# arnaucube/go-snark-study

Hardware: AMD Instinct MI355X
Metric: Groth16 constraints/sec (prove) at 2^20 R1CS (higher is better)
Workload: dtype u32 (9x29-bit Montgomery limbs of the 254-bit BN128 fields)

## Files before the change

### __graft_entry__.py

```python
import os
import subprocess
import sys

ROOT = os.path.dirname(os.path.abspath(__file__))
if ROOT not in sys.path:
    sys.path.insert(0, ROOT)
TESTS = os.path.join(ROOT, "tests")


def build():
    jobs = str(min(8, os.cpu_count() or 1))
    subprocess.check_call(["make", "-s", "-j", jobs, "-C", os.path.join(ROOT, "go-snark-study_amd", "csrc")])
    subprocess.check_call(["make", "-s", "-C", os.path.join(ROOT, "oracle")])
    prim_src = os.path.join(ROOT, "tests", "device", "prim_test.hip")
    prim_lib = os.path.join(ROOT, "tests", "device", "libgs_prim_test.so")
    hdrs = [os.path.join(ROOT, "go-snark-study_amd", "csrc", h) for h in ("fp29.h", "fq2.h", "ec.h", "point_io.h")]
    hdrs.append(os.path.join(ROOT, "tests", "device", "limit_ops.h"))
    if not os.path.exists(prim_lib) or os.path.getmtime(prim_lib) < max(os.path.getmtime(f) for f in [prim_src] + hdrs):
        subprocess.check_call(["hipcc", "--offload-arch=gfx950", "-O3", "-std=c++17", "-fPIC", "-shared", "-Wno-unused-function", prim_src, "-o", prim_lib])
    if os.path.isdir("/root/reference"):
        subprocess.check_call(["make", "-s", "-C", os.path.join(ROOT, "oracle"), "ref"])
    import gosnark_amd
    from gosnark_amd import capi
    capi.load_library()
    _stamp_build()
    return None


def _stamp_build():
    import hashlib
    import json
    lib = os.path.join(ROOT, "go-snark-study_amd", "libgosnark_hip.so")
    info = {"lib_sha256": hashlib.sha256(open(lib, "rb").read()).hexdigest()}
    try:
        info["commit"] = subprocess.check_output(["git", "-C", ROOT, "rev-parse", "HEAD"], stderr=subprocess.DEVNULL).decode().strip()
        dirty = subprocess.check_output(["git", "-C", ROOT, "status", "--porcelain", "--", "go-snark-study_amd/csrc", "include"],
                                        stderr=subprocess.DEVNULL).decode()
        info["sources_modified_since_commit"] = sorted(line[3:] for line in dirty.splitlines() if len(line) > 3)
    except (OSError, subprocess.CalledProcessError):
        return
    with open(os.path.join(ROOT, "go-snark-study_amd", "BUILD_INFO.json"), "w") as f:
        json.dump(info, f, indent=1)


def smoke():
    import numpy as np
    import torch
    assert torch.cuda.is_available(), "smoke() needs a GPU"
    torch.cuda.set_device(0)
    if TESTS not in sys.path:
        sys.path.insert(0, TESTS)
    import gosnark_amd
    from gosnark_amd import capi, groth16
    capi.init(0)
    import golden_util as GU
    import gpu_util as U
    from oracle import c_oracle as C
    from oracle import ref_py as O
    rec = GU.load("groth_x3")
    opk = GU.groth_pk(rec["setup"])
    r, s = GU.rs_from_stream(rec["rand"])
    circ = groth16.Circuit(rec["circuit"]["NVars"], rec["circuit"]["NPublic"])
    pk = groth16.Pk(BACDelta=opk.BACDelta, Z=opk.Z, G1_Alpha=opk.G1_Alpha, G1_Beta=opk.G1_Beta, G1_Delta=opk.G1_Delta,
                    G1_At=opk.G1_At, G1_BACGamma=opk.G1_BACGamma, G2_Beta=opk.G2_Beta, G2_Delta=opk.G2_Delta,
                    G2_BACGamma=opk.G2_BACGamma, PowersTauDelta=opk.PowersTauDelta)
    proof = groth16.GenerateProofsWithRS(circ, pk, rec["w"], rec["px"], r, s)
    a = O.G1.Affine(GU.g1(rec["proof"]["PiA"]))
    b = O.G2.Affine(GU.g2(rec["proof"]["PiB"]))
    c = O.G1.Affine(GU.g1(rec["proof"]["PiC"]))
    assert proof.PiA == (a[0], a[1], 1), "PiA differs from the reference prover"
    assert proof.PiB == (b[0], b[1], (1, 0)), "PiB differs from the reference prover"
    assert proof.PiC == (c[0], c[1], 1), "PiC differs from the reference prover"
    n = 4096
    ks = U.rand_scalars_u64(n, 11)
    bases = capi.g1_fixed_base(ks)
    pts = capi.g1_download(bases)
    sc = U.rand_scalars_u64(n, 12)
    got = capi.msm(bases, sc)
    want = C.g1_affine(C.g1_msm_naive(pts, sc, threads=min(8, os.cpu_count() or 1)))
    assert got == want, "G1 MSM (table-free route) differs from the oracle's naive MulScalar/Add loop"
    capi.build_tables(bases)
    assert capi.handle_bytes(bases)[1] > 0 and capi.msm(bases, sc) == want, "G1 MSM (window-table route) differs from the oracle"
    proof2 = groth16.GenerateProofsWithRS(circ, pk, rec["w"], rec["px"], r, s)
    assert (proof2.PiA, proof2.PiB, proof2.PiC) == (proof.PiA, proof.PiB, proof.PiC)
    print("smoke ok: groth16 x^3+x+5 proof == reference wasm proof (affine); 4096-term G1 MSM == oracle on both summation routes;",
          capi.version())
    return None


if __name__ == "__main__":
    build()
    if len(sys.argv) > 1 and sys.argv[1] == "smoke":
        smoke()
```

### go-snark-study_amd/csrc/msm.hip

```cpp
#include "msm.h"
#include "hostcopy.h"

#include <algorithm>
#include <cmath>
#include <cstdlib>
#include <future>
#include <type_traits>

#include "msm_kernels.h"

namespace gs {

static_assert(sizeof(G1Xyzz) == PointIO<FqTag>::kXyzzWords * 4, "G1 XYZZ must be raw limbs");
static_assert(sizeof(G2Xyzz) == PointIO<Fq2Tag>::kXyzzWords * 4, "G2 XYZZ must be raw limbs");

static inline dim3 grid1(size_t n, int block = 256) { return dim3((unsigned)((n + block - 1) / block)); }

int choose_window_bits(uint32_t n, int forced) {
  if (forced >= 8 && forced <= kMaxWindowBits) return forced;
  static const double per_bucket = dev_knob_f("GS_WINDOW_COST_BUCKET", 6.0, 0.0, 64.0);
  static const int auto_max = (int)dev_knob("GS_AUTO_MAX_C", 17, 8, kMaxWindowBits);
  int best = 8;
  double best_cost = 1e300;
  for (int c = 8; c <= std::min(kMaxWindowBits, std::max(8, auto_max)); ++c) {
    const int W = 254 / c + 1;
    const double cost = (double)n * W + per_bucket * (double)(1u << (c - 1));
    if (cost < best_cost) { best_cost = cost; best = c; }
  }
  return best;
}

int choose_window_bits_free(uint32_t n, int forced) {
  if (forced) return std::min(kMaxFreeWindowBits, std::max(kMinFreeWindowBits, forced));
  static const double per_bucket = dev_knob_f("GS_WINDOW_COST_BUCKET_FREE", 3.0, 0.0, 64.0);
  int best = kMinFreeWindowBits;
  double best_cost = 1e300;
  for (int c = kMinFreeWindowBits; c <= kMaxFreeWindowBits; ++c) {
    const int W = 254 / c + 1;
    const double cost = (double)W * ((double)n + per_bucket * (double)(1u << (c - 1)));
    if (cost < best_cost) { best_cost = cost; best = c; }
  }
  return best;
}

static void exclusive_scan(Ctx& c, PlanBuffers& pb, const uint32_t* in, uint32_t* out, uint32_t n) {
  const uint32_t ntiles = (n + kScanTile - 1) / kScanTile;
  pb.tiles.ensure((size_t)ntiles * 4);
  pb.total.ensure(4);
  hipLaunchKernelGGL(k_scan_tiles, dim3(ntiles), dim3(kScanBlock), 0, c.stream, in, out, pb.tiles.as<uint32_t>(), n);
  hipLaunchKernelGGL(k_scan_tile_sums, dim3(1), dim3(1024), 0, c.stream, pb.tiles.as<uint32_t>(), ntiles, pb.total.as<uint32_t>());
  hipLaunchKernelGGL(k_scan_add, dim3(ntiles), dim3(kScanBlock), 0, c.stream, out, pb.tiles.as<uint32_t>(), n);
}

struct MsmState {
  PlanBuffers plan_slots[3 * Ctx::kSlots];
  DevBuf table_scratch;
  DevBuf table_scratch_bg;
  DevBuf upload_scratch;
  DevBuf upload_flag;
  bool lds_attr_set = false;
};
static MsmState& msm_state(Ctx& c) { return c.state<MsmState>(c.msm_state); }

static uint32_t choose_chunk(uint64_t entries, uint32_t nbuckets, const std::vector<LaunchShape>& users) {
  static const int forced = (int)dev_knob("GS_CHUNK", 0, 4, 1024, 4);
  if (forced >= 4 && forced % 4 == 0) return (uint32_t)forced;
  static const int forced_h = (int)dev_knob("GS_CHUNK_H", 0, 4, 1024, 4);
  if (forced_h && users.size() == 1 && users[0].njobs == 1 && !users[0].g2) return (uint32_t)forced_h;
  uint32_t chunk = entries >= (1ull << 27) ? 64u : entries >= (1ull << 23) ? 32u : 16u;
  while (chunk < 1024u && entries / std::max<uint32_t>(nbuckets, 1u) > 32ull * chunk) chunk *= 2;
  return chunk;
}

static uint32_t part_min_ranges() {
  static const uint32_t v = (uint32_t)dev_knob("GS_PART_MIN_R", 4, 2, 64);
  return v;
}
bool plan_partitions_first(int cbits) {
  if (cbits < 1) return false;
  return std::max<uint32_t>(1u, (1u << (cbits - 1)) >> kRangeLog) >= part_min_ranges();
}

uint32_t finite_mask_dev(Ctx& c, const uint32_t* g1_pts, const uint32_t* g2_pts, uint32_t n, uint32_t* mask_dev) {
  const size_t words = ((size_t)n + 31) / 32;
  GS_HIP(hipMemsetAsync(mask_dev, 0, std::max<size_t>(words, 1) * 4, c.stream));
  DevBuf cnt(4);
  GS_HIP(hipMemsetAsync(cnt.p, 0, 4, c.stream));
  if (n) hipLaunchKernelGGL(k_finite_mask, grid1(n), dim3(256), 0, c.stream, g1_pts, (uint32_t)PointIO<FqTag>::kAffineWords, g2_pts,
                            (uint32_t)PointIO<Fq2Tag>::kAffineWords, n, mask_dev, cnt.as<uint32_t>());
  GS_HIP(hipGetLastError());
  uint32_t host = 0;
  GS_HIP(hipMemcpyAsync(&host, cnt.p, 4, hipMemcpyDeviceToHost, c.stream));
  GS_HIP(hipStreamSynchronize(c.stream));
  return host;
}

void build_plan(Ctx& c, int slot, const uint32_t* scalars_dev, uint32_t n, MsmPlan& plan, const std::vector<LaunchShape>& users, int cbits,
                bool table_free, const uint32_t* term_index, uint32_t index_bias) {
  MsmState& ms = msm_state(c);
  PlanBuffers& pb = ms.plan_slots[slot % (3 * Ctx::kSlots)];
  plan.n = n;
  plan.table_free = table_free;
  plan.c = cbits ? cbits : (table_free ? choose_window_bits_free(n, c.window_bits) : choose_window_bits(n, c.window_bits));
  if (table_free && (plan.c < kMinFreeWindowBits || plan.c > kMaxFreeWindowBits))
    throw HipError{hipErrorInvalidValue, "table-free plan outside 9..16 window bits", __LINE__};
  plan.W = 254 / plan.c + 1;
  plan.B = 1u << (plan.c - 1);
  plan.nbuckets = table_free ? (uint32_t)plan.W * plan.B : plan.B;
  plan.chunk = choose_chunk((uint64_t)n * plan.W, plan.nbuckets, users);
  plan.maxchunks = (uint32_t)(((size_t)n * plan.W + plan.chunk - 1) / plan.chunk) + 1;
  const size_t ncount = (size_t)plan.nbuckets + 1;
  PlanParams pp{};
  pp.n = n; pp.c = plan.c; pp.W = plan.W; pp.B = plan.B;
  pp.R = std::max<uint32_t>(1u, plan.B >> kRangeLog);
  pp.tf = table_free ? 1u : 0u;
  {
    const uint32_t want = std::max<uint32_t>(1u, 256u / (plan.W * pp.R));
    const uint32_t by_size = std::max<uint32_t>(1u, (n + 16383u) / 16384u);
    const uint32_t by_mem = std::max<uint32_t>(1u, (uint32_t)((64ull << 20) / ((uint64_t)plan.B * plan.W * 4)));
    pp.S = std::max<uint32_t>(1u, std::min(std::min<uint32_t>(16u, std::max<uint32_t>(want, 1u)), std::min(by_size, by_mem)));
    if (pp.R == 1 && !table_free) pp.S = std::max<uint32_t>(1u, std::min<uint32_t>(16u, by_size));
  }
  pp.slice = (n + pp.S - 1) / pp.S;
  pp.stride = (n + 63u) & ~63u;
  const bool wide = plan_partitions_first(plan.c);
  if (wide && term_index) throw HipError{hipErrorInvalidValue, "plans over a term list cannot be sorted partition-first (plan_partitions_first)", __LINE__};
  const uint32_t nparts = (uint32_t)plan.W * pp.R;
  if (wide && nparts > kMaxParts) throw HipError{hipErrorInvalidValue, "too many (window, range) partitions", __LINE__};
  if (!wide) pb.digits.ensure((size_t)std::max<uint32_t>(pp.stride, 64u) * plan.W * sizeof(digit_t));
  else {
    pb.recs.ensure(std::max<size_t>((size_t)n * plan.W, 1) * 8);
    pb.parts.ensure((size_t)(3 * kMaxParts + 4) * 4);
  }
  pb.hist.ensure((size_t)plan.B * plan.W * pp.S * 4);
  pb.totals.ensure(ncount * 4);
  pb.offsets.ensure(ncount * 4);
  pb.entries.ensure(((size_t)plan.maxchunks + 1) * plan.chunk * 4);
  pb.chunk_bucket.ensure((size_t)plan.maxchunks * 4);
  pb.heavy_list.ensure((size_t)plan.nbuckets * 4);
  pb.counters.ensure(16);
  const size_t lds = (size_t)std::min<uint32_t>(plan.B, kRangeBuckets) * 4;
  static const int sort_block = (int)dev_knob("GS_SORT_BLOCK", kSortBlock, 64, kSortBlock, 64);
  if (!ms.lds_attr_set) {
    GS_HIP(hipFuncSetAttribute(reinterpret_cast<const void*>(k_hist), hipFuncAttributeMaxDynamicSharedMemorySize, 128 * 1024));
    GS_HIP(hipFuncSetAttribute(reinterpret_cast<const void*>(k_scatter), hipFuncAttributeMaxDynamicSharedMemorySize, 128 * 1024));
    GS_HIP(hipFuncSetAttribute(reinterpret_cast<const void*>(k_hist_part), hipFuncAttributeMaxDynamicSharedMemorySize, 128 * 1024));
    GS_HIP(hipFuncSetAttribute(reinterpret_cast<const void*>(k_scatter_part), hipFuncAttributeMaxDynamicSharedMemorySize, 128 * 1024));
    ms.lds_attr_set = true;
  }
  GS_HIP(hipMemsetAsync(pb.totals.as<uint32_t>() + plan.nbuckets, 0, 4, c.stream));
  GS_HIP(hipMemsetAsync(pb.counters.p, 0, 16, c.stream));
  uint32_t* part_count = pb.parts.as<uint32_t>();
  uint32_t* part_base = part_count ? part_count + kMaxParts : nullptr;
  uint32_t* part_cursor = part_count ? part_base + kMaxParts + 4 : nullptr;
  if (n > 0 && wide) {
    GS_HIP(hipMemsetAsync(part_count, 0, (size_t)nparts * 4, c.stream));
    hipLaunchKernelGGL(k_part_count, grid1(n, kPartBlock), dim3(kPartBlock), 0, c.stream, scalars_dev, pp, part_count);
    hipLaunchKernelGGL(k_part_scan, dim3(1), dim3(64), 0, c.stream, part_count, nparts, part_base, part_cursor);
    hipLaunchKernelGGL(k_part_scatter, grid1(n, kPartBlock * kPartPerThread), dim3(kPartBlock), 0, c.stream, scalars_dev, pp, part_base, part_cursor,
                       pb.recs.as<uint2>());
    hipLaunchKernelGGL(k_hist_part, dim3(8 * pp.S * ((nparts + 7) / 8)), dim3(sort_block), lds, c.stream, pb.recs.as<uint2>(), part_base, pp, pb.hist.as<uint32_t>());
    hipLaunchKernelGGL(k_colscan, grid1(plan.B), dim3(256), 0, c.stream, pb.hist.as<uint32_t>(), pp, pb.totals.as<uint32_t>());
  } else if (n > 0) {
    hipLaunchKernelGGL(k_digits, grid1(n), dim3(256), 0, c.stream, scalars_dev, pp, pb.digits.as<digit_t>(), term_index, index_bias);
    hipLaunchKernelGGL(k_hist, dim3(plan.W, pp.S, pp.R), dim3(sort_block), lds, c.stream, pb.digits.as<digit_t>(), pp, pb.hist.as<uint32_t>());
    if (table_free) hipLaunchKernelGGL(k_colscan_windows, grid1(plan.nbuckets), dim3(256), 0, c.stream, pb.hist.as<uint32_t>(), pp, pb.totals.as<uint32_t>());
    else hipLaunchKernelGGL(k_colscan, grid1(plan.B), dim3(256), 0, c.stream, pb.hist.as<uint32_t>(), pp, pb.totals.as<uint32_t>());
  } else {
    GS_HIP(hipMemsetAsync(pb.totals.p, 0, ncount * 4, c.stream));
  }
  exclusive_scan(c, pb, pb.totals.as<uint32_t>(), pb.offsets.as<uint32_t>(), (uint32_t)ncount);
  if (n > 0) {
    if (wide) hipLaunchKernelGGL(k_scatter_part, dim3(8 * pp.S * ((nparts + 7) / 8)), dim3(sort_block), lds, c.stream, pb.recs.as<uint2>(), part_base, pp,
                                 pb.hist.as<uint32_t>(), pb.offsets.as<uint32_t>(), pb.entries.as<uint32_t>());
    else hipLaunchKernelGGL(k_scatter, dim3(plan.W, pp.S, pp.R), dim3(sort_block), lds, c.stream, pb.digits.as<digit_t>(), pp, pb.hist.as<uint32_t>(),
                            pb.offsets.as<uint32_t>(), pb.entries.as<uint32_t>(), term_index, index_bias);
    hipLaunchKernelGGL(k_chunk_map, grid1(plan.nbuckets), dim3(256), 0, c.stream, pb.offsets.as<uint32_t>(), plan.nbuckets, plan.chunk,
                       pb.chunk_bucket.as<uint32_t>(), pb.heavy_list.as<uint32_t>(), pb.counters.as<uint32_t>());
  }
  GS_HIP(hipGetLastError());
  plan.offsets = pb.offsets.as<uint32_t>();
  plan.entries = pb.entries.as<uint32_t>();
  plan.chunk_bucket = pb.chunk_bucket.as<uint32_t>();
  plan.heavy_list = pb.heavy_list.as<uint32_t>();
  plan.heavy_count = pb.counters.as<uint32_t>();
}

template <class T>
static void enqueue_table_slabs(hipStream_t stream, DevBuf& scratch, const uint32_t* src, size_t n, int cbits, DevBuf& rows, size_t first, size_t last,
                                size_t slab) {
  const int W = 254 / cbits + 1;
  if (first >= last) return;
  static const bool per_row = dev_flag("GS_TABLE_PER_ROW");
  if (per_row || W <= 2) {
    if (first == 0) hipLaunchKernelGGL(k_build_table<T>, grid1(n), dim3(256), 0, stream, src, (uint32_t)n, cbits, W, rows.as<uint32_t>());
  } else {
    constexpr size_t sw = PointIO<T>::kXyzzWords + PointIO<T>::kXyzzWords / 4;
    slab = std::min<size_t>(std::max<size_t>(slab, 1), n);
    scratch.ensure(slab * (size_t)(W - 1) * sw * 4);
    for (size_t at = first; at < last; at += slab) {
      const size_t count = std::min(slab, last - at);
      hipLaunchKernelGGL(k_build_table_batched<T>, grid1(count), dim3(256), 0, stream, src, (uint32_t)n, (uint32_t)at, (uint32_t)count, cbits, W,
                         rows.as<uint32_t>(), scratch.as<uint32_t>());
    }
  }
  GS_HIP(hipGetLastError());
}
template <class T>
static void enqueue_table_build(Ctx& c, hipStream_t stream, DevBuf& scratch, const uint32_t* src, size_t n, int cbits, DevBuf& fresh,
                                size_t slab_max = (size_t)1 << 18) {
  constexpr size_t aw = PointIO<T>::kAffineWords;
  const int W = 254 / cbits + 1;
  fresh.alloc(std::max<size_t>(n, 1) * W * aw * 4);
  enqueue_table_slabs<T>(stream, scratch, src, n, cbits, fresh, 0, n, slab_max);
}

template <class T>
static void ensure_table(Ctx& c, BaseTable& t, const uint32_t* row0, size_t n, int cbits) {
  if (t.c == cbits && t.n == n && t.rows.p) return;
  table_settle(c, t, false);
  const uint32_t* src = row0 ? row0 : t.rows.as<uint32_t>();
  if (!src || (!row0 && t.n != n)) throw HipError{hipErrorInvalidValue, "window table rebuild without its points", __LINE__};
  DevBuf fresh;
  enqueue_table_build<T>(c, c.stream, msm_state(c).table_scratch, src, n, cbits, fresh);
  GS_HIP(hipStreamSynchronize(c.stream));
  t.rows = std::move(fresh);
  t.n = n; t.c = cbits; t.W = 254 / cbits + 1;
  t.uses = 0;
}
void ensure_table_g1(Ctx& c, BaseTable& t, const uint32_t* row0, size_t n, int cbits) { ensure_table<FqTag>(c, t, row0, n, cbits); }
void ensure_table_g2(Ctx& c, BaseTable& t, const uint32_t* row0, size_t n, int cbits) { ensure_table<Fq2Tag>(c, t, row0, n, cbits); }

constexpr uint32_t kTableAfterUses = 2;

template <class T>
static void enqueue_pending_slabs(Ctx& c, BaseTable& t, size_t first, size_t last, size_t slab) {
  enqueue_table_slabs<T>(c.main_stream, msm_state(c).table_scratch_bg, t.pending_src, t.pending_n, t.pending_c, t.pending, first, last, slab);
}
static size_t instalment_slab(size_t n, bool g2) {
  static const size_t cap = (size_t)1 << run_knob("GS_TABLE_BG_SLAB_LOG2", 18, 10, 18);
  return std::min(g2 ? std::max<size_t>(cap / 2, (size_t)1 << 12) : cap, std::max<size_t>(n, 1));
}
static void order_streams_behind(Ctx& c, hipEvent_t ev) {
  for (auto a : c.aux_stream) if (a && a != c.main_stream) GS_HIP(hipStreamWaitEvent(a, ev, 0));
}

void table_settle(Ctx& c, BaseTable& t, bool install) {
  if (!t.pending.p) return;
  if (install && !t.pending_complete()) {
    const size_t slab = (size_t)1 << 18;
    if (t.pending_g2) enqueue_pending_slabs<Fq2Tag>(c, t, t.pending_next, t.pending_n, slab);
    else enqueue_pending_slabs<FqTag>(c, t, t.pending_next, t.pending_n, slab);
    t.pending_next = t.pending_n;
    GS_HIP(hipEventRecord(t.pending_done, c.main_stream));
  }
  if (t.pending_done && t.pending_next > 0) GS_HIP(hipEventSynchronize(t.pending_done));
  else if (t.pending_next > 0) GS_HIP(hipStreamSynchronize(c.main_stream));
  if (install) {
    t.rows = std::move(t.pending);
    t.n = t.pending_n; t.c = t.pending_c; t.W = 254 / t.pending_c + 1;
    t.uses = 0;
  } else t.pending.release();
  t.pending_c = 0; t.pending_n = 0; t.pending_next = 0; t.pending_src = nullptr;
}

static void install_enqueued(Ctx& c, BaseTable& t) {
  if (hipEventQuery(t.pending_done) != hipSuccess) order_streams_behind(c, t.pending_done);
  (void)hipGetLastError();
  t.rows = std::move(t.pending);
  t.n = t.pending_n; t.c = t.pending_c; t.W = 254 / t.pending_c + 1;
  t.uses = 0;
  t.pending_c = 0; t.pending_n = 0; t.pending_next = 0; t.pending_src = nullptr;
}

static bool begin_pending(Ctx& c, BaseTable& t, const TableRef& r, int cbits) {
  if (!t.pending_done) GS_HIP(hipEventCreateWithFlags(&t.pending_done, hipEventDisableTiming));
  const int W = 254 / cbits + 1;
  const size_t aw = r.g2 ? PointIO<Fq2Tag>::kAffineWords : PointIO<FqTag>::kAffineWords;
  try {
    constexpr size_t sw2 = PointIO<Fq2Tag>::kXyzzWords + PointIO<Fq2Tag>::kXyzzWords / 4;
    if (W > 2) {
      constexpr size_t sw1 = PointIO<FqTag>::kXyzzWords + PointIO<FqTag>::kXyzzWords / 4;
      const size_t s2 = instalment_slab(r.n, true), s1 = instalment_slab(r.n, false);
      const size_t bytes = std::max((s2 + s2 / 4) * sw2, (s1 + s1 / 4) * sw1);
      msm_state(c).table_scratch_bg.ensure(bytes * (size_t)(W - 1) * 4);
    }
    t.pending.alloc(std::max<size_t>(r.n, 1) * W * aw * 4);
  } catch (const HipError& e) {
    if (e.e != hipErrorOutOfMemory) throw;
    t.pending.release();
    return false;
  }
  t.pending_c = cbits; t.pending_n = r.n; t.pending_next = 0; t.pending_src = r.row0; t.pending_g2 = r.g2;
  return true;
}

static bool advance_pending(Ctx& c, BaseTable& t, double& credit) {
  const double unit = t.pending_g2 ? kG2BuildCost : 1.0;
  const size_t slab = instalment_slab(t.pending_n, t.pending_g2);
  for (;;) {
    if (t.pending_next >= t.pending_n) break;
    const size_t last = t.pending_n - t.pending_next <= slab + slab / 4 ? t.pending_n : t.pending_next + slab;
    if (credit < 0.5 * (double)(last - t.pending_next) * unit) break;
    if (t.pending_g2) enqueue_pending_slabs<Fq2Tag>(c, t, t.pending_next, last, last - t.pending_next);
    else enqueue_pending_slabs<FqTag>(c, t, t.pending_next, last, last - t.pending_next);
    credit -= (double)(last - t.pending_next) * unit;
    t.pending_next = last;
  }
  if (t.pending_next < t.pending_n) return false;
  GS_HIP(hipEventRecord(t.pending_done, c.main_stream));
  return true;
}

void stamp_tables(Ctx& c, const std::vector<BaseTable*>& tables) {
  for (BaseTable* t : tables) if (t) t->last_use = c.call_clock;
}

bool prepare_tables(Ctx& c, const std::vector<TableRef>& group, uint32_t nterms, int* cbits, double* credit) {
  int cb = choose_window_bits(std::max<uint32_t>(nterms, 1u), c.window_bits);
  if (c.window_bits == 0 && !group.empty() && group[0].t->rows.p) {
    const int tc = group[0].t->c;
    bool same = tc >= cb - 1 && tc <= cb + 1;
    for (const TableRef& r : group) same = same && r.t->ready(r.n, tc);
    if (same) cb = tc;
  }
  bool all_ready = true;
  for (const TableRef& r : group) {
// ... 358 lines not shown
```

### go-snark-study_amd/csrc/msm_kernels.h

```cpp
#pragma once
#include <hip/hip_runtime.h>
#include <stdint.h>

#include "ec.h"
#include "point_io.h"

namespace gs {

struct PlanParams {
  uint32_t n;
  int c;
  int W;
  uint32_t B;
  uint32_t S;
  uint32_t slice;
  uint32_t stride;
  uint32_t R;
  uint32_t tf;
};
constexpr uint32_t kRangeLog = 15;
constexpr uint32_t kRangeBuckets = 1u << kRangeLog;

GS_HD int32_t next_digit(const uint32_t (&k)[8], const PlanParams& pp, int w, uint32_t& carry) {
  uint32_t raw = scalar_bits(k, w * pp.c, pp.c) + carry;
  if (raw > pp.B) { carry = 1; return (int32_t)raw - (int32_t)(2u * pp.B); }
  carry = 0;
  return (int32_t)raw;
}

using digit_t = uint32_t;
__global__ void __launch_bounds__(256) k_digits(const uint32_t* __restrict__ scalars, PlanParams pp, digit_t* __restrict__ digits,
                                                 const uint32_t* __restrict__ term_index, uint32_t index_bias) {
  wave_priority<GS_PRIO_PLAN>();
  const uint32_t i = blockIdx.x * blockDim.x + threadIdx.x;
  if (i >= pp.n) return;
  const uint32_t src = term_index ? term_index[i] - index_bias : i;
  uint32_t k[8];
  const uint4* s4 = reinterpret_cast<const uint4*>(scalars + (size_t)src * 8);
  uint4 lo = s4[0], hi = s4[1];
  k[0] = lo.x; k[1] = lo.y; k[2] = lo.z; k[3] = lo.w; k[4] = hi.x; k[5] = hi.y; k[6] = hi.z; k[7] = hi.w;
  scalar_canon(k);
  uint32_t carry = 0;
  for (int w = 0; w < pp.W; ++w) {
    const int32_t d = next_digit(k, pp, w, carry);
    digits[(size_t)w * pp.stride + i] = (digit_t)(d + (int32_t)pp.B - 1);
  }
}

__global__ void __launch_bounds__(256) k_finite_mask(const uint32_t* __restrict__ a, uint32_t wa, const uint32_t* __restrict__ b, uint32_t wb, uint32_t n,
                                                      uint32_t* __restrict__ mask, uint32_t* __restrict__ count) {
  const uint32_t i = blockIdx.x * blockDim.x + threadIdx.x;
  bool finite = false;
  if (i < n) {
    uint32_t acc = 0;
    if (a) for (uint32_t k = 0; k < wa; ++k) acc |= a[(size_t)i * wa + k];
    if (b) for (uint32_t k = 0; k < wb; ++k) acc |= b[(size_t)i * wb + k];
    finite = acc != 0;
  }
  if (finite) { atomicOr(&mask[i >> 5], 1u << (i & 31u)); atomicAdd(count, 1u); }
}

constexpr int kSortBlock = 1024;

__global__ void __launch_bounds__(kSortBlock) k_hist(const digit_t* __restrict__ digits, PlanParams pp, uint32_t* __restrict__ hist) {
  wave_priority<GS_PRIO_PLAN>();
  extern __shared__ uint32_t sh[];
  const uint32_t w = blockIdx.x, s = blockIdx.y, r = blockIdx.z;
  const uint32_t nb = min(pp.B, kRangeBuckets), base = r << kRangeLog;
  for (uint32_t b = threadIdx.x; b < nb; b += blockDim.x) sh[b] = 0;
  __syncthreads();
  const uint32_t lo = s * pp.slice, hi = min(pp.n, lo + pp.slice);
  const digit_t* row = digits + (size_t)w * pp.stride;
  const int32_t zero = (int32_t)pp.B - 1;
  for (uint32_t i = lo + threadIdx.x; i < hi; i += blockDim.x) {
    const int32_t d = (int32_t)row[i] - zero;
    if (d != 0) {
      const uint32_t b = (uint32_t)(d < 0 ? -d : d) - 1u;
      if ((b >> kRangeLog) == r) atomicAdd(&sh[b - base], 1u);
    }
  }
  __syncthreads();
  uint32_t* out = hist + ((size_t)w * pp.S + s) * pp.B + base;
  for (uint32_t b = threadIdx.x; b < nb; b += blockDim.x) out[b] = sh[b];
}

__global__ void __launch_bounds__(256) k_colscan(uint32_t* __restrict__ hist, PlanParams pp, uint32_t* __restrict__ totals) {
  wave_priority<GS_PRIO_PLAN>();
  const uint32_t b = blockIdx.x * blockDim.x + threadIdx.x;
  if (b >= pp.B) return;
  uint32_t* col = hist + b;
  const uint32_t nq = (uint32_t)pp.W * pp.S;
  uint32_t run = 0;
  for (uint32_t q = 0; q < nq; ++q) { const uint32_t t = col[(size_t)q * pp.B]; col[(size_t)q * pp.B] = run; run += t; }
  totals[b] = run;
}

__global__ void __launch_bounds__(256) k_colscan_windows(uint32_t* __restrict__ hist, PlanParams pp, uint32_t* __restrict__ totals) {
  wave_priority<GS_PRIO_PLAN>();
  const uint32_t i = blockIdx.x * blockDim.x + threadIdx.x;
  if (i >= (uint32_t)pp.W * pp.B) return;
  const uint32_t w = i / pp.B, b = i % pp.B;
  uint32_t* col = hist + (size_t)w * pp.S * pp.B + b;
  uint32_t run = 0;
  for (uint32_t q = 0; q < pp.S; ++q) { const uint32_t t = col[(size_t)q * pp.B]; col[(size_t)q * pp.B] = run; run += t; }
  totals[i] = run;
}

__global__ void __launch_bounds__(kSortBlock) k_scatter(const digit_t* __restrict__ digits, PlanParams pp, const uint32_t* __restrict__ hist,
                                                         const uint32_t* __restrict__ offsets, uint32_t* __restrict__ entries,
                                                         const uint32_t* __restrict__ term_index, uint32_t index_bias) {
  wave_priority<GS_PRIO_PLAN>();
  extern __shared__ uint32_t sh[];
  const uint32_t w = blockIdx.x, s = blockIdx.y, r = blockIdx.z;
  const uint32_t nb = min(pp.B, kRangeBuckets), base = r << kRangeLog;
  const uint32_t* pre = hist + ((size_t)w * pp.S + s) * pp.B + base;
  const uint32_t* off = offsets + (pp.tf ? (size_t)w * pp.B : (size_t)0);
  for (uint32_t b = threadIdx.x; b < nb; b += blockDim.x) sh[b] = off[base + b] + pre[b];
  __syncthreads();
  const uint32_t lo = s * pp.slice, hi = min(pp.n, lo + pp.slice);
  const digit_t* row = digits + (size_t)w * pp.stride;
  const int32_t zero = (int32_t)pp.B - 1;
  for (uint32_t i = lo + threadIdx.x; i < hi; i += blockDim.x) {
    const int32_t d = (int32_t)row[i] - zero;
    if (d != 0) {
      const uint32_t b = (uint32_t)(d < 0 ? -d : d) - 1u;
      if ((b >> kRangeLog) == r) {
        const uint32_t pos = atomicAdd(&sh[b - base], 1u);
        const uint32_t id = term_index ? term_index[i] - index_bias : i;
        entries[pos] = id | (w << kWindowShift) | (d < 0 ? kSignBit : 0u);
      }
    }
  }
}

constexpr int kPartBlock = 256;
constexpr int kPartPerThread = 4;
constexpr uint32_t kMaxParts = 512;

GS_HD void load_scalar_canon(const uint32_t* __restrict__ scalars, uint32_t i, uint32_t (&k)[8]) {
  const uint4* s4 = reinterpret_cast<const uint4*>(scalars + (size_t)i * 8);
  const uint4 lo = s4[0], hi = s4[1];
  k[0] = lo.x; k[1] = lo.y; k[2] = lo.z; k[3] = lo.w; k[4] = hi.x; k[5] = hi.y; k[6] = hi.z; k[7] = hi.w;
  scalar_canon(k);
}

__global__ void __launch_bounds__(kPartBlock) k_part_count(const uint32_t* __restrict__ scalars, PlanParams pp, uint32_t* __restrict__ part_count) {
  wave_priority<GS_PRIO_PLAN>();
  __shared__ uint32_t cnt[kMaxParts];
  const uint32_t nparts = (uint32_t)pp.W * pp.R;
  for (uint32_t t = threadIdx.x; t < nparts; t += kPartBlock) cnt[t] = 0;
  __syncthreads();
  const uint32_t i = blockIdx.x * kPartBlock + threadIdx.x;
  if (i < pp.n) {
    uint32_t k[8];
    load_scalar_canon(scalars, i, k);
    uint32_t carry = 0;
    for (int w = 0; w < pp.W; ++w) {
      const int32_t d = next_digit(k, pp, w, carry);
      if (d != 0) atomicAdd(&cnt[(uint32_t)w * pp.R + (((uint32_t)(d < 0 ? -d : d) - 1u) >> kRangeLog)], 1u);
    }
  }
  __syncthreads();
  for (uint32_t t = threadIdx.x; t < nparts; t += kPartBlock) if (cnt[t]) atomicAdd(&part_count[t], cnt[t]);
}

__global__ void __launch_bounds__(64) k_part_scan(uint32_t* __restrict__ part_count, uint32_t nparts, uint32_t* __restrict__ part_base,
                                                    uint32_t* __restrict__ part_cursor) {
  wave_priority<GS_PRIO_PLAN>();
  if (blockIdx.x != 0 || threadIdx.x != 0) return;
  uint32_t run = 0;
  for (uint32_t t = 0; t < nparts; ++t) { part_base[t] = run; run += part_count[t]; part_cursor[t] = 0; part_count[t] = 0; }
  part_base[nparts] = run;
}

__global__ void __launch_bounds__(kPartBlock) k_part_scatter(const uint32_t* __restrict__ scalars, PlanParams pp, const uint32_t* __restrict__ part_base,
                                                              uint32_t* __restrict__ part_cursor, uint2* __restrict__ recs) {
  wave_priority<GS_PRIO_PLAN>();
  __shared__ uint32_t cnt[kMaxParts];
  const uint32_t nparts = (uint32_t)pp.W * pp.R;
  for (uint32_t t = threadIdx.x; t < nparts; t += kPartBlock) cnt[t] = 0;
  __syncthreads();
  const uint32_t first = blockIdx.x * (kPartBlock * kPartPerThread);
  for (int j = 0; j < kPartPerThread; ++j) {
    const uint32_t i = first + j * kPartBlock + threadIdx.x;
    if (i >= pp.n) break;
    uint32_t k[8];
    load_scalar_canon(scalars, i, k);
    uint32_t carry = 0;
    for (int w = 0; w < pp.W; ++w) {
      const int32_t d = next_digit(k, pp, w, carry);
      if (d != 0) atomicAdd(&cnt[(uint32_t)w * pp.R + (((uint32_t)(d < 0 ? -d : d) - 1u) >> kRangeLog)], 1u);
    }
  }
  __syncthreads();
  for (uint32_t t = threadIdx.x; t < nparts; t += kPartBlock) {
    const uint32_t mine = cnt[t];
    cnt[t] = part_base[t] + (mine ? atomicAdd(&part_cursor[t], mine) : 0u);
  }
  __syncthreads();
  for (int j = 0; j < kPartPerThread; ++j) {
    const uint32_t i = first + j * kPartBlock + threadIdx.x;
    if (i >= pp.n) break;
    uint32_t k[8];
    load_scalar_canon(scalars, i, k);
    uint32_t carry = 0;
    for (int w = 0; w < pp.W; ++w) {
      const int32_t d = next_digit(k, pp, w, carry);
      if (d != 0) {
        const uint32_t b = (uint32_t)(d < 0 ? -d : d) - 1u;
        const uint32_t pos = atomicAdd(&cnt[(uint32_t)w * pp.R + (b >> kRangeLog)], 1u);
        recs[pos] = make_uint2(i | (d < 0 ? kSignBit : 0u), b);
      }
    }
  }
}

GS_HD bool part_of_block(uint32_t id, const PlanParams& pp, uint32_t& w, uint32_t& r, uint32_t& s) {
  const uint32_t xcd = id & 7u, j = id >> 3;
  const uint32_t p = xcd + 8u * (j / pp.S);
  s = j % pp.S;
  w = p / pp.R; r = p % pp.R;
  return p < (uint32_t)pp.W * pp.R;
}

GS_HD void part_slice(const uint32_t* __restrict__ part_base, const PlanParams& pp, uint32_t w, uint32_t r, uint32_t s, uint32_t& lo, uint32_t& hi) {
  const uint32_t p0 = part_base[w * pp.R + r], p1 = part_base[w * pp.R + r + 1];
  const uint32_t len = p1 - p0, per = (len + pp.S - 1) / pp.S;
  lo = min(p1, p0 + s * per);
  hi = min(p1, lo + per);
}

__global__ void __launch_bounds__(kSortBlock) k_hist_part(const uint2* __restrict__ recs, const uint32_t* __restrict__ part_base, PlanParams pp,
                                                           uint32_t* __restrict__ hist) {
  wave_priority<GS_PRIO_PLAN>();
  extern __shared__ uint32_t sh[];
  uint32_t w, r, s;
  if (!part_of_block(blockIdx.x, pp, w, r, s)) return;
  const uint32_t base = r << kRangeLog;
  for (uint32_t b = threadIdx.x; b < kRangeBuckets; b += blockDim.x) sh[b] = 0;
  __syncthreads();
  uint32_t lo, hi;
  part_slice(part_base, pp, w, r, s, lo, hi);
  for (uint32_t e = lo + threadIdx.x; e < hi; e += blockDim.x) atomicAdd(&sh[recs[e].y - base], 1u);
  __syncthreads();
  uint32_t* out = hist + ((size_t)w * pp.S + s) * pp.B + base;
  for (uint32_t b = threadIdx.x; b < kRangeBuckets; b += blockDim.x) out[b] = sh[b];
}

__global__ void __launch_bounds__(kSortBlock) k_scatter_part(const uint2* __restrict__ recs, const uint32_t* __restrict__ part_base, PlanParams pp,
                                                              const uint32_t* __restrict__ hist, const uint32_t* __restrict__ offsets,
                                                              uint32_t* __restrict__ entries) {
  wave_priority<GS_PRIO_PLAN>();
  extern __shared__ uint32_t sh[];
  uint32_t w, r, s;
  if (!part_of_block(blockIdx.x, pp, w, r, s)) return;
  const uint32_t base = r << kRangeLog;
  const uint32_t* pre = hist + ((size_t)w * pp.S + s) * pp.B + base;
  for (uint32_t b = threadIdx.x; b < kRangeBuckets; b += blockDim.x) sh[b] = offsets[base + b] + pre[b];
  __syncthreads();
  uint32_t lo, hi;
  part_slice(part_base, pp, w, r, s, lo, hi);
  for (uint32_t e = lo + threadIdx.x; e < hi; e += blockDim.x) {
    const uint2 rec = recs[e];
    entries[atomicAdd(&sh[rec.y - base], 1u)] = rec.x | (w << kWindowShift);
  }
}

constexpr int kScanBlock = 256;
constexpr int kScanPerThread = 8;
constexpr int kScanTile = kScanBlock * kScanPerThread;

__global__ void __launch_bounds__(kScanBlock) k_scan_tiles(const uint32_t* __restrict__ in, uint32_t* __restrict__ out,
                                                            uint32_t* __restrict__ tile_sums, uint32_t n) {
  wave_priority<GS_PRIO_PLAN>();
  __shared__ uint32_t sh[kScanBlock];
  const uint32_t base = blockIdx.x * kScanTile + threadIdx.x * kScanPerThread;
  uint32_t v[kScanPerThread], sum = 0;
#pragma unroll
  for (int j = 0; j < kScanPerThread; ++j) { v[j] = (base + j < n) ? in[base + j] : 0u; sum += v[j]; }
  sh[threadIdx.x] = sum;
  __syncthreads();
  for (int off = 1; off < kScanBlock; off <<= 1) {
    uint32_t t = (threadIdx.x >= (uint32_t)off) ? sh[threadIdx.x - off] : 0u;
    __syncthreads();
    sh[threadIdx.x] += t;
    __syncthreads();
  }
  uint32_t run = sh[threadIdx.x] - sum;
#pragma unroll
  for (int j = 0; j < kScanPerThread; ++j) { if (base + j < n) out[base + j] = run; run += v[j]; }
  if (threadIdx.x == kScanBlock - 1) tile_sums[blockIdx.x] = sh[threadIdx.x];
}

__global__ void __launch_bounds__(1024) k_scan_tile_sums(uint32_t* __restrict__ tile_sums, uint32_t ntiles, uint32_t* __restrict__ total) {
  wave_priority<GS_PRIO_PLAN>();
  __shared__ uint32_t sh[1024];
  const uint32_t per = (ntiles + 1023u) / 1024u;
  const uint32_t b0 = threadIdx.x * per;
  uint32_t sum = 0;
  for (uint32_t j = 0; j < per; ++j) if (b0 + j < ntiles) sum += tile_sums[b0 + j];
  sh[threadIdx.x] = sum;
  __syncthreads();
  for (int off = 1; off < 1024; off <<= 1) {
    uint32_t t = (threadIdx.x >= (uint32_t)off) ? sh[threadIdx.x - off] : 0u;
    __syncthreads();
    sh[threadIdx.x] += t;
    __syncthreads();
  }
  uint32_t run = sh[threadIdx.x] - sum;
  for (uint32_t j = 0; j < per; ++j) if (b0 + j < ntiles) { uint32_t t = tile_sums[b0 + j]; tile_sums[b0 + j] = run; run += t; }
  if (threadIdx.x == 1023) *total = sh[1023];
}

__global__ void __launch_bounds__(kScanBlock) k_scan_add(uint32_t* __restrict__ out, const uint32_t* __restrict__ tile_sums, uint32_t n) {
  wave_priority<GS_PRIO_PLAN>();
  const uint32_t base = blockIdx.x * kScanTile + threadIdx.x * kScanPerThread;
  const uint32_t add = tile_sums[blockIdx.x];
#pragma unroll
  for (int j = 0; j < kScanPerThread; ++j) if (base + j < n) out[base + j] += add;
}

constexpr uint32_t kHeavySpan = 64;

__global__ void __launch_bounds__(256) k_chunk_map(const uint32_t* __restrict__ offsets, uint32_t nbuckets, uint32_t chunk,
                                                    uint32_t* __restrict__ chunk_bucket, uint32_t* __restrict__ heavy_list,
                                                    uint32_t* __restrict__ heavy_count) {
  wave_priority<GS_PRIO_PLAN>();
  const uint32_t b = blockIdx.x * blockDim.x + threadIdx.x;
  if (b >= nbuckets) return;
  const uint32_t o0 = offsets[b], o1 = offsets[b + 1];
  if (o1 == o0) return;
  const uint32_t t0 = (o0 + chunk - 1) / chunk, t1 = (o1 + chunk - 1) / chunk;
  for (uint32_t t = t0; t < t1; ++t) chunk_bucket[t] = b;
  if ((o1 - 1) / chunk - o0 / chunk > kHeavySpan) {
    heavy_list[atomicAdd(heavy_count, 1u)] = b;
  }
}

struct AccJob {
  const uint32_t* table;
  uint32_t row_stride;
  uint32_t* buckets;
  uint32_t* heads;
  uint32_t* tails;
  uint32_t* merged;
  uint32_t* out;
  uint32_t* final_out;
};
constexpr int kMaxJobs = 8;
struct AccJobs { AccJob j[kMaxJobs]; };

template <class T> struct AccTuning;
#ifndef GS_G1_WAVES
#define GS_G1_WAVES 3
#endif
#ifndef GS_G1_PREFETCH
#define GS_G1_PREFETCH 1
#endif
#ifndef GS_G2_TOUCH
#define GS_G2_TOUCH 0
#endif
template <> struct AccTuning<FqTag> { static constexpr int kMinWaves = GS_G1_WAVES; static constexpr bool kRegisterPrefetch = GS_G1_PREFETCH != 0; static constexpr bool kTouch = true; };
#ifndef GS_G2_WAVES
#define GS_G2_WAVES 2
#endif
#ifndef GS_G2_PREFETCH
#define GS_G2_PREFETCH 0
#endif
template <> struct AccTuning<Fq2Tag> { static constexpr int kMinWaves = GS_G2_WAVES; static constexpr bool kRegisterPrefetch = GS_G2_PREFETCH != 0; static constexpr bool kTouch = GS_G2_TOUCH != 0; };

#ifndef GS_ACC_BLOCK
#define GS_ACC_BLOCK 256
#endif
constexpr int kAccBlock = GS_ACC_BLOCK;
template <class T>
__global__ void __launch_bounds__(kAccBlock, AccTuning<T>::kMinWaves) k_bucket_accumulate(AccJobs jobs, const uint32_t* __restrict__ offsets,
                                                            const uint32_t* __restrict__ entries,
                                                            const uint32_t* __restrict__ chunk_bucket, uint32_t nbuckets, uint32_t chunk) {
  constexpr int pw = PointIO<T>::kXyzzWords;
  constexpr int aw = PointIO<T>::kAffineWords;
  const uint32_t t = blockIdx.x * blockDim.x + threadIdx.x;
  const uint32_t total = offsets[nbuckets];
  const uint32_t beg = t * chunk;
  if (beg >= total) return;
  const uint32_t end = min(beg + chunk, total);
  const AccJob job = jobs.j[blockIdx.y];
  uint32_t b = chunk_bucket[t];
  uint32_t bend = offsets[b + 1];
  bool started_before = offsets[b] < beg;
  constexpr bool kTight = GS_PAIR != 0 && T::kWords != 8;
  using Acc = std::conditional_t<kTight, XyzzAcc<T>, Xyzz<T>>;
  auto acc_inf = [] { if constexpr (kTight) return xyzz_acc_inf<T>(); else return xyzz_inf<T>(); };
  auto acc_store = [](uint32_t* p, const Acc& a) { if constexpr (kTight) store_xyzz<T>(p, to_xyzz(a)); else store_xyzz<T>(p, a); };
  Acc acc = acc_inf();
  const uint4* e4 = reinterpret_cast<const uint4*>(entries + beg);
  constexpr bool kPre = AccTuning<T>::kRegisterPrefetch;
  uint4 q = e4[0];
  uint32_t v = q.x;
  uint32_t nb = b;
  const uint32_t* np = job.table + ((size_t)((v >> kWindowShift) & 31u) * job.row_stride + (v & kIndexMask)) * aw;
  RawAffine<T> nextp;
  uint32_t touch = 0;
  if constexpr (kPre) nextp = load_raw_affine<T>(np);
  for (uint32_t e = beg; e < end; ++e) {
    const uint32_t cur = v;
    const uint32_t* cp = np;
    RawAffine<T> curp;
    if constexpr (kPre) curp = nextp;
    if (e >= bend) {
      acc_store((started_before ? job.heads + (size_t)t * pw : job.buckets + (size_t)b * pw), acc);
      started_before = false;
      acc = acc_inf();
      b = nb; bend = offsets[b + 1];
    }
    if (e + 1 < end) {
      const uint32_t k = (e + 1 - beg) & 3u;
      if (k == 0) q = e4[(e + 1 - beg) >> 2];
      v = k == 0 ? q.x : k == 1 ? q.y : k == 2 ? q.z : q.w;
// ... 390 lines not shown
```

Baseline: 131.9 million.

## Plan MSM buckets slice-major from scalars and scan offsets in one block

For table-backed plans with few bucket ranges, the planner now reads the scalars directly in per-slice histogram and scatter kernels. Each thread recomputes all window digits in-register, so the materialised digits array and the per-window histogram layout are no longer needed. A single-block 1024-thread exclusive scan replaces the multi-kernel scan and the two memsets when the bucket count is small enough. This is meant to cut planning kernel launches and memory traffic, at the cost of recomputing digits twice and serialising the scan in one workgroup.

```diff
diff --git a/__graft_entry__.py b/__graft_entry__.py
--- a/__graft_entry__.py
+++ b/__graft_entry__.py
@@ -18,6 +18,13 @@
     hdrs.append(os.path.join(ROOT, "tests", "device", "limit_ops.h"))
     if not os.path.exists(prim_lib) or os.path.getmtime(prim_lib) < max(os.path.getmtime(f) for f in [prim_src] + hdrs):
         subprocess.check_call(["hipcc", "--offload-arch=gfx950", "-O3", "-std=c++17", "-fPIC", "-shared", "-Wno-unused-function", prim_src, "-o", prim_lib])
+    plan_src = os.path.join(ROOT, "tests", "device", "plan_test.hip")
+    plan_lib = os.path.join(ROOT, "tests", "device", "libgs_plan_test.so")
+    csrc = os.path.join(ROOT, "go-snark-study_amd", "csrc")
+    plan_deps = [plan_src] + [os.path.join(csrc, h) for h in os.listdir(csrc) if h.endswith(".h")]
+    if not os.path.exists(plan_lib) or os.path.getmtime(plan_lib) < max(os.path.getmtime(f) for f in plan_deps):
+        subprocess.check_call(["hipcc", "--offload-arch=gfx950", "-O3", "-std=c++17", "-fPIC", "-shared", "-fvisibility=hidden", "-Wno-unused-function",
+                               plan_src, "-o", plan_lib])
     if os.path.isdir("/root/reference"):
         subprocess.check_call(["make", "-s", "-C", os.path.join(ROOT, "oracle"), "ref"])
     import gosnark_amd
diff --git a/go-snark-study_amd/csrc/msm.hip b/go-snark-study_amd/csrc/msm.hip
--- a/go-snark-study_amd/csrc/msm.hip
+++ b/go-snark-study_amd/csrc/msm.hip
@@ -124,15 +124,21 @@
   pp.slice = (n + pp.S - 1) / pp.S;
   pp.stride = (n + 63u) & ~63u;
   const bool wide = plan_partitions_first(plan.c);
+  static const bool by_window = dev_flag("GS_PLAN_BY_WINDOW");
+  static const bool scan3 = dev_flag("GS_PLAN_SCAN3");
+  const bool slice_major = !table_free && !wide && pp.R <= 2 && !by_window;
+  if (slice_major) {
+    const SliceShape shape = plan_slice_shape(n, plan.B);
+    pp.S = shape.S; pp.slice = shape.slice;
+  }
   if (wide && term_index) throw HipError{hipErrorInvalidValue, "plans over a term list cannot be sorted partition-first (plan_partitions_first)", __LINE__};
   const uint32_t nparts = (uint32_t)plan.W * pp.R;
   if (wide && nparts > kMaxParts) throw HipError{hipErrorInvalidValue, "too many (window, range) partitions", __LINE__};
-  if (!wide) pb.digits.ensure((size_t)std::max<uint32_t>(pp.stride, 64u) * plan.W * sizeof(digit_t));
-  else {
+  if (wide) {
     pb.recs.ensure(std::max<size_t>((size_t)n * plan.W, 1) * 8);
     pb.parts.ensure((size_t)(3 * kMaxParts + 4) * 4);
-  }
-  pb.hist.ensure((size_t)plan.B * plan.W * pp.S * 4);
+  } else if (!slice_major) pb.digits.ensure((size_t)std::max<uint32_t>(pp.stride, 64u) * plan.W * sizeof(digit_t));
+  pb.hist.ensure((size_t)plan.B * (slice_major ? 1u : (uint32_t)plan.W) * pp.S * 4);
   pb.totals.ensure(ncount * 4);
   pb.offsets.ensure(ncount * 4);
   pb.entries.ensure(((size_t)plan.maxchunks + 1) * plan.chunk * 4);
@@ -146,10 +152,15 @@
     GS_HIP(hipFuncSetAttribute(reinterpret_cast<const void*>(k_scatter), hipFuncAttributeMaxDynamicSharedMemorySize, 128 * 1024));
     GS_HIP(hipFuncSetAttribute(reinterpret_cast<const void*>(k_hist_part), hipFuncAttributeMaxDynamicSharedMemorySize, 128 * 1024));
     GS_HIP(hipFuncSetAttribute(reinterpret_cast<const void*>(k_scatter_part), hipFuncAttributeMaxDynamicSharedMemorySize, 128 * 1024));
+    slice_sort_lds_attributes();
+    GS_HIP(hipGetLastError());
     ms.lds_attr_set = true;
   }
-  GS_HIP(hipMemsetAsync(pb.totals.as<uint32_t>() + plan.nbuckets, 0, 4, c.stream));
-  GS_HIP(hipMemsetAsync(pb.counters.p, 0, 16, c.stream));
+  const bool scan_one = slice_major && !scan3 && ncount <= kScanOneMax;
+  if (!scan_one) {
+    GS_HIP(hipMemsetAsync(pb.totals.as<uint32_t>() + plan.nbuckets, 0, 4, c.stream));
+    GS_HIP(hipMemsetAsync(pb.counters.p, 0, 16, c.stream));
+  }
   uint32_t* part_count = pb.parts.as<uint32_t>();
   uint32_t* part_base = part_count ? part_count + kMaxParts : nullptr;
   uint32_t* part_cursor = part_count ? part_base + kMaxParts + 4 : nullptr;
@@ -160,19 +171,24 @@
     hipLaunchKernelGGL(k_part_scatter, grid1(n, kPartBlock * kPartPerThread), dim3(kPartBlock), 0, c.stream, scalars_dev, pp, part_base, part_cursor,
                        pb.recs.as<uint2>());
     hipLaunchKernelGGL(k_hist_part, dim3(8 * pp.S * ((nparts + 7) / 8)), dim3(sort_block), lds, c.stream, pb.recs.as<uint2>(), part_base, pp, pb.hist.as<uint32_t>());
-    hipLaunchKernelGGL(k_colscan, grid1(plan.B), dim3(256), 0, c.stream, pb.hist.as<uint32_t>(), pp, pb.totals.as<uint32_t>());
+    hipLaunchKernelGGL(k_colscan, grid1(plan.B), dim3(256), 0, c.stream, pb.hist.as<uint32_t>(), pp, (uint32_t)plan.W * pp.S, pb.totals.as<uint32_t>());
+  } else if (n > 0 && slice_major) {
+    enqueue_slice_hist(c.stream, scalars_dev, pp, pb.hist.as<uint32_t>(), pb.totals.as<uint32_t>(), term_index, index_bias, sort_block);
   } else if (n > 0) {
     hipLaunchKernelGGL(k_digits, grid1(n), dim3(256), 0, c.stream, scalars_dev, pp, pb.digits.as<digit_t>(), term_index, index_bias);
     hipLaunchKernelGGL(k_hist, dim3(plan.W, pp.S, pp.R), dim3(sort_block), lds, c.stream, pb.digits.as<digit_t>(), pp, pb.hist.as<uint32_t>());
     if (table_free) hipLaunchKernelGGL(k_colscan_windows, grid1(plan.nbuckets), dim3(256), 0, c.stream, pb.hist.as<uint32_t>(), pp, pb.totals.as<uint32_t>());
-    else hipLaunchKernelGGL(k_colscan, grid1(plan.B), dim3(256), 0, c.stream, pb.hist.as<uint32_t>(), pp, pb.totals.as<uint32_t>());
+    else hipLaunchKernelGGL(k_colscan, grid1(plan.B), dim3(256), 0, c.stream, pb.hist.as<uint32_t>(), pp, (uint32_t)plan.W * pp.S, pb.totals.as<uint32_t>());
   } else {
     GS_HIP(hipMemsetAsync(pb.totals.p, 0, ncount * 4, c.stream));
   }
-  exclusive_scan(c, pb, pb.totals.as<uint32_t>(), pb.offsets.as<uint32_t>(), (uint32_t)ncount);
+  if (scan_one) enqueue_scan_one(c.stream, pb.totals.as<uint32_t>(), pb.offsets.as<uint32_t>(), (uint32_t)ncount, pb.counters.as<uint32_t>());
+  else exclusive_scan(c, pb, pb.totals.as<uint32_t>(), pb.offsets.as<uint32_t>(), (uint32_t)ncount);
   if (n > 0) {
     if (wide) hipLaunchKernelGGL(k_scatter_part, dim3(8 * pp.S * ((nparts + 7) / 8)), dim3(sort_block), lds, c.stream, pb.recs.as<uint2>(), part_base, pp,
                                  pb.hist.as<uint32_t>(), pb.offsets.as<uint32_t>(), pb.entries.as<uint32_t>());
+    else if (slice_major) enqueue_slice_scatter(c.stream, scalars_dev, pp, pb.hist.as<uint32_t>(), pb.offsets.as<uint32_t>(), pb.entries.as<uint32_t>(),
+                                                term_index, index_bias, sort_block);
     else hipLaunchKernelGGL(k_scatter, dim3(plan.W, pp.S, pp.R), dim3(sort_block), lds, c.stream, pb.digits.as<digit_t>(), pp, pb.hist.as<uint32_t>(),
                             pb.offsets.as<uint32_t>(), pb.entries.as<uint32_t>(), term_index, index_bias);
     hipLaunchKernelGGL(k_chunk_map, grid1(plan.nbuckets), dim3(256), 0, c.stream, pb.offsets.as<uint32_t>(), plan.nbuckets, plan.chunk,
diff --git a/go-snark-study_amd/csrc/msm_kernels.h b/go-snark-study_amd/csrc/msm_kernels.h
--- a/go-snark-study_amd/csrc/msm_kernels.h
+++ b/go-snark-study_amd/csrc/msm_kernels.h
@@ -84,12 +84,11 @@
   for (uint32_t b = threadIdx.x; b < nb; b += blockDim.x) out[b] = sh[b];
 }
 
-__global__ void __launch_bounds__(256) k_colscan(uint32_t* __restrict__ hist, PlanParams pp, uint32_t* __restrict__ totals) {
+__global__ void __launch_bounds__(256) k_colscan(uint32_t* __restrict__ hist, PlanParams pp, uint32_t nq, uint32_t* __restrict__ totals) {
   wave_priority<GS_PRIO_PLAN>();
   const uint32_t b = blockIdx.x * blockDim.x + threadIdx.x;
   if (b >= pp.B) return;
   uint32_t* col = hist + b;
-  const uint32_t nq = (uint32_t)pp.W * pp.S;
   uint32_t run = 0;
   for (uint32_t q = 0; q < nq; ++q) { const uint32_t t = col[(size_t)q * pp.B]; col[(size_t)q * pp.B] = run; run += t; }
   totals[b] = run;
@@ -264,6 +263,170 @@
     const uint2 rec = recs[e];
     entries[atomicAdd(&sh[rec.y - base], 1u)] = rec.x | (w << kWindowShift);
   }
+}
+
+constexpr uint32_t kPlanRound = 256;
+constexpr uint32_t kSliceMin = kSortBlock;
+constexpr uint32_t kSliceAlign = 64;
+constexpr uint64_t kHistBytesMax = 64ull << 20;
+
+struct SliceShape {
+  uint32_t S;
+  uint32_t slice;
+  uint32_t R;
+};
+inline SliceShape plan_slice_shape(uint32_t n, uint32_t B) {
+  SliceShape sh;
+  sh.R = B > kRangeBuckets ? B >> kRangeLog : 1u;
+  const uint32_t by_round = kPlanRound / sh.R > 0 ? kPlanRound / sh.R : 1u;
+  const uint64_t by_mem = kHistBytesMax / ((uint64_t)B * 4) > 0 ? kHistBytesMax / ((uint64_t)B * 4) : 1u;
+  const uint32_t by_size = n > kSliceMin ? (uint32_t)(((uint64_t)n + kSliceMin - 1) / kSliceMin) : 1u;
+  uint32_t S = by_size < by_round ? by_size : by_round;
+  if ((uint64_t)S > by_mem) S = (uint32_t)by_mem;
+  if (S >= 8u) S &= ~7u;
+  sh.S = S;
+  const uint64_t per = ((uint64_t)n + S - 1) / S;
+  sh.slice = (uint32_t)((per + kSliceAlign - 1) / kSliceAlign * kSliceAlign);
+  if (sh.slice == 0) sh.slice = kSliceAlign;
+  return sh;
+}
+GS_HD uint32_t slice_of_block(uint32_t x, uint32_t S) { return (S & 7u) ? x : (x & 7u) * (S >> 3) + (x >> 3); }
+
+__global__ void __launch_bounds__(kSortBlock) k_hist_slices(const uint32_t* __restrict__ scalars, PlanParams pp, uint32_t* __restrict__ hist,
+                                                             const uint32_t* __restrict__ term_index, uint32_t index_bias) {
+  wave_priority<GS_PRIO_PLAN>();
+  extern __shared__ uint32_t sh[];
+  const uint32_t s = slice_of_block(blockIdx.x, pp.S), r = blockIdx.y;
+  const uint32_t nb = min(pp.B, kRangeBuckets), base = r << kRangeLog;
+  for (uint32_t b = threadIdx.x; b < nb; b += blockDim.x) sh[b] = 0;
+  __syncthreads();
+  const uint32_t lo = min(pp.n, s * pp.slice), hi = min(pp.n, lo + pp.slice);
+  for (uint32_t i = lo + threadIdx.x; i < hi; i += blockDim.x) {
+    const uint32_t id = term_index ? term_index[i] - index_bias : i;
+    uint32_t k[8];
+    load_scalar_canon(scalars, id, k);
+    uint32_t carry = 0;
+    for (int w = 0; w < pp.W; ++w) {
+      const int32_t d = next_digit(k, pp, w, carry);
+      if (d != 0) {
+        const uint32_t b = (uint32_t)(d < 0 ? -d : d) - 1u;
+        if ((b >> kRangeLog) == r) atomicAdd(&sh[b - base], 1u);
+      }
+    }
+  }
+  __syncthreads();
+  uint32_t* out = hist + (size_t)s * pp.B + base;
+  for (uint32_t b = threadIdx.x; b < nb; b += blockDim.x) out[b] = sh[b];
+}
+
+__global__ void __launch_bounds__(kSortBlock) k_scatter_slices(const uint32_t* __restrict__ scalars, PlanParams pp, const uint32_t* __restrict__ hist,
+                                                                const uint32_t* __restrict__ offsets, uint32_t* __restrict__ entries,
+                                                                const uint32_t* __restrict__ term_index, uint32_t index_bias) {
+  wave_priority<GS_PRIO_PLAN>();
+  extern __shared__ uint32_t sh[];
+  const uint32_t s = slice_of_block(blockIdx.x, pp.S), r = blockIdx.y;
+  const uint32_t nb = min(pp.B, kRangeBuckets), base = r << kRangeLog;
+  const uint32_t* pre = hist + (size_t)s * pp.B + base;
+  for (uint32_t b = threadIdx.x; b < nb; b += blockDim.x) sh[b] = offsets[base + b] + pre[b];
+  __syncthreads();
+  const uint32_t lo = min(pp.n, s * pp.slice), hi = min(pp.n, lo + pp.slice);
+  for (uint32_t i = lo + threadIdx.x; i < hi; i += blockDim.x) {
+    const uint32_t id = term_index ? term_index[i] - index_bias : i;
+    uint32_t k[8];
+    load_scalar_canon(scalars, id, k);
+    uint32_t carry = 0;
+    for (int w = 0; w < pp.W; ++w) {
+      const int32_t d = next_digit(k, pp, w, carry);
+      if (d != 0) {
+        const uint32_t b = (uint32_t)(d < 0 ? -d : d) - 1u;
+        if ((b >> kRangeLog) == r) entries[atomicAdd(&sh[b - base], 1u)] = id | ((uint32_t)w << kWindowShift) | (d < 0 ? kSignBit : 0u);
+      }
+    }
+  }
+}
+
+constexpr int kScanOneGroups = 17;
+constexpr uint32_t kScanOneMax = (uint32_t)kScanOneGroups * 4096u;
+
+__global__ void __launch_bounds__(1024) k_scan_one(const uint32_t* __restrict__ in, uint32_t* __restrict__ out, uint32_t n,
+                                                    uint32_t* __restrict__ counters) {
+  wave_priority<GS_PRIO_PLAN>();
+  __shared__ uint32_t wsum[kScanOneGroups * 16];
+  __shared__ uint32_t gsum[kScanOneGroups];
+  const uint32_t t = threadIdx.x, lane = t & 63u, wv = t >> 6;
+  if (t == 0 && counters) { counters[0] = 0; counters[1] = 0; counters[2] = 0; counters[3] = 0; }
+  const uint32_t last = n ? n - 1u : 0u;
+  auto load4 = [&](int g, uint32_t (&v)[4]) {
+    const uint32_t i0 = (uint32_t)g * 4096u + t * 4u;
+    if (i0 + 4u <= last) {
+      const uint4 q = *reinterpret_cast<const uint4*>(in + i0);
+      v[0] = q.x; v[1] = q.y; v[2] = q.z; v[3] = q.w;
+    } else {
+#pragma unroll
+      for (int j = 0; j < 4; ++j) v[j] = (i0 + j < last) ? in[i0 + j] : 0u;
+    }
+  };
+  uint32_t x[kScanOneGroups];
+#pragma unroll
+  for (int g = 0; g < kScanOneGroups; ++g) {
+    uint32_t v[4];
+    load4(g, v);
+    x[g] = v[0] + v[1] + v[2] + v[3];
+  }
+#pragma unroll
+  for (int g = 0; g < kScanOneGroups; ++g) {
+    uint32_t inc = x[g];
+#pragma unroll
+    for (int off = 1; off < 64; off <<= 1) { const uint32_t u = __shfl_up(inc, off, 64); if (lane >= (uint32_t)off) inc += u; }
+    if (lane == 63u) wsum[g * 16 + wv] = inc;
+    x[g] = inc - x[g];
+  }
+  __syncthreads();
+  if (t < (uint32_t)kScanOneGroups) {
+    uint32_t run = 0;
+    for (int k = 0; k < 16; ++k) { const uint32_t u = wsum[t * 16 + k]; wsum[t * 16 + k] = run; run += u; }
+    gsum[t] = run;
+  }
+  __syncthreads();
+  if (t == 0) {
+    uint32_t run = 0;
+    for (int g = 0; g < kScanOneGroups; ++g) { const uint32_t u = gsum[g]; gsum[g] = run; run += u; }
+  }
+  __syncthreads();
+#pragma unroll
+  for (int g = 0; g < kScanOneGroups; ++g) {
+    const uint32_t i0 = (uint32_t)g * 4096u + t * 4u;
+    uint32_t v[4];
+    load4(g, v);
+    uint32_t run = gsum[g] + wsum[g * 16 + wv] + x[g];
+    if (i0 + 4u <= n) {
+      uint4 q;
+      q.x = run; q.y = run + v[0]; q.z = q.y + v[1]; q.w = q.z + v[2];
+      *reinterpret_cast<uint4*>(out + i0) = q;
+    } else {
+#pragma unroll
+      for (int j = 0; j < 4; ++j) { if (i0 + j < n) out[i0 + j] = run; run += v[j]; }
+    }
+  }
+}
+
+inline void slice_sort_lds_attributes() {
+  (void)hipFuncSetAttribute(reinterpret_cast<const void*>(k_hist_slices), hipFuncAttributeMaxDynamicSharedMemorySize, 128 * 1024);
+  (void)hipFuncSetAttribute(reinterpret_cast<const void*>(k_scatter_slices), hipFuncAttributeMaxDynamicSharedMemorySize, 128 * 1024);
+}
+inline void enqueue_slice_hist(hipStream_t stream, const uint32_t* scalars, const PlanParams& pp, uint32_t* hist, uint32_t* totals,
+                               const uint32_t* term_index, uint32_t index_bias, int block) {
+  const size_t lds = (size_t)(pp.B < kRangeBuckets ? pp.B : kRangeBuckets) * 4;
+  hipLaunchKernelGGL(k_hist_slices, dim3(pp.S, pp.R), dim3(block), lds, stream, scalars, pp, hist, term_index, index_bias);
+  hipLaunchKernelGGL(k_colscan, dim3((pp.B + 255u) / 256u), dim3(256), 0, stream, hist, pp, pp.S, totals);
+}
+inline void enqueue_scan_one(hipStream_t stream, const uint32_t* totals, uint32_t* offsets, uint32_t ncount, uint32_t* counters) {
+  hipLaunchKernelGGL(k_scan_one, dim3(1), dim3(1024), 0, stream, totals, offsets, ncount, counters);
+}
+inline void enqueue_slice_scatter(hipStream_t stream, const uint32_t* scalars, const PlanParams& pp, const uint32_t* hist, const uint32_t* offsets,
+                                  uint32_t* entries, const uint32_t* term_index, uint32_t index_bias, int block) {
+  const size_t lds = (size_t)(pp.B < kRangeBuckets ? pp.B : kRangeBuckets) * 4;
+  hipLaunchKernelGGL(k_scatter_slices, dim3(pp.S, pp.R), dim3(block), lds, stream, scalars, pp, hist, offsets, entries, term_index, index_bias);
 }
 
 constexpr int kScanBlock = 256;
```

After: 131.6 million. No clear change (-0.2%).
